# jynik/OOKiedokie

Hardware: NVIDIA B200
Metric: IQ Msamples/s decoded (SC16Q11->OOK msgs) (higher is better)
Workload: dtype f32

## Files before the change

### ookiedokie_b200/csrc/screen_tma.cuh

```cuda
#pragma once

#include <cuda.h>

#include "fir_kernels.cuh"

namespace ookd {

struct ScreenTmaArgs {
    ScreenArgs s;
    i64 row0_sample;
    uint32_t fast_lo, fast_hi;
};

constexpr int STMA_NT = 256, STMA_SPT = 16, STMA_L = STMA_NT * STMA_SPT;
constexpr int STMA_STAGES = 3;
constexpr int STMA_BODY = STMA_L * 4;
constexpr int STMA8_BOX_ROWS = 8;
constexpr int STMA_HT_MAX = 5;
constexpr int STMA_HIST = 384;
constexpr int STMA_XY_ROWS = STMA_NT + STMA_HT_MAX;
constexpr int STMA_SMEM_BYTES = STMA_STAGES * STMA_BODY + STMA_STAGES * STMA_HIST + STMA_STAGES * STMA_XY_ROWS * 8 + 32;
constexpr int STMA_TUNE_BYTES = 528;
static_assert(4 * (STMA_SMEM_BYTES + STMA_TUNE_BYTES + 1024) <= 228 * 1024, "four CTAs per SM");

#ifndef OOKD_STMA_L2_HINT
#define OOKD_STMA_L2_HINT 0x12F0000000000000ull
#endif
#ifndef OOKD_STMA_MINB
#define OOKD_STMA_MINB 4
#endif

__device__ __forceinline__ uint32_t smem_u32(const void *p)
{
    return (uint32_t) __cvta_generic_to_shared(p);
}

__device__ __forceinline__ void mbar_init(uint32_t bar, uint32_t count)
{
    asm volatile("mbarrier.init.shared::cta.b64 [%0], %1;" ::"r"(bar), "r"(count) : "memory");
}

__device__ __forceinline__ void mbar_expect_tx(uint32_t bar, uint32_t bytes)
{
    asm volatile("mbarrier.arrive.expect_tx.shared::cta.b64 _, [%0], %1;" ::"r"(bar), "r"(bytes) : "memory");
}

__device__ __forceinline__ void mbar_wait(uint32_t bar, uint32_t parity)
{
    asm volatile(
        "{\n\t"
        ".reg .pred p;\n\t"
        "WAIT_%=:\n\t"
        "mbarrier.try_wait.parity.shared::cta.b64 p, [%0], %1;\n\t"
        "@p bra DONE_%=;\n\t"
        "bra WAIT_%=;\n\t"
        "DONE_%=:\n\t"
        "}" ::"r"(bar), "r"(parity) : "memory");
}

__device__ __forceinline__ void tma_load_tile(uint32_t dst, const CUtensorMap *map, int32_t row, uint32_t bar)
{
    asm volatile(
        "cp.async.bulk.tensor.2d.shared::cluster.global.mbarrier::complete_tx::bytes.L2::cache_hint"
        " [%0], [%1, {%3, %4}], [%2], %5;" ::"r"(dst), "l"((uint64_t) map), "r"(bar), "r"(0), "r"(row),
        "l"(OOKD_STMA_L2_HINT)
        : "memory");
}

__device__ __forceinline__ uint4 lds128(uint32_t addr)
{
    uint4 v;
    asm volatile("ld.shared.v4.u32 {%0,%1,%2,%3}, [%4];" : "=r"(v.x), "=r"(v.y), "=r"(v.z), "=r"(v.w) : "r"(addr));
    return v;
}

__device__ __forceinline__ void sts128(uint32_t addr, uint32_t a, uint32_t b, uint32_t c, uint32_t d)
{
    asm volatile("st.shared.v4.u32 [%0], {%1,%2,%3,%4};" ::"r"(addr), "r"(a), "r"(b), "r"(c), "r"(d) : "memory");
}

__device__ __forceinline__ int stma_chunk_off(int u, int v)
{
    const int R = u >> 1;
    return R * 128 + (((((u & 1) << 2) | v) ^ (R & 7)) << 4);
}

__device__ __forceinline__ int dp2a_lo_s16_u8(uint32_t a, uint32_t b, int c)
{
    int d;
    asm("dp2a.lo.s32.u32 %0, %1, %2, %3;" : "=r"(d) : "r"(a), "r"(b), "r"(c));
    return d;
}

__device__ __forceinline__ int dp2a_hi_s16_s8(uint32_t a, uint32_t b, int c)
{
    int d;
    asm("dp2a.hi.s32.s32 %0, %1, %2, %3;" : "=r"(d) : "r"(a), "r"(b), "r"(c));
    return d;
}

__device__ __forceinline__ void screen_span_energy(const uint32_t (&w)[16], uint32_t (&pre)[16], uint32_t &hi_total)
{
    int lo = 0, hi = 0;
#pragma unroll
    for (int e = 0; e < 16; e++) {
        const uint32_t b = __byte_perm(w[e], 0u, 0x3120);
        lo = dp2a_lo_s16_u8(w[e], b, lo);
        hi = dp2a_hi_s16_s8(w[e], b, hi);
        pre[e] = (uint32_t) (lo + (hi << 8));
    }
    hi_total = (uint32_t) hi;
}

__device__ __forceinline__ void screen_span_sums(const uint32_t (&w)[16], int &sx, int &sy)
{
    int xs = 0, ys = 0;
#pragma unroll
    for (int e = 0; e < 16; e++) {
        xs += (int) (short) (w[e] & 0xFFFFu);
        ys += ((int) w[e]) >> 16;
    }
    sx = xs;
    sy = ys;
}

#define OOKD_XY_QUIET ((int) 0x80000000)

__device__ __forceinline__ void screen_span_stats_v2(const uint32_t (&w)[16], uint32_t (&pre)[16], int &sx, int &sy, uint32_t &tot,
                                                     uint32_t k0)
{
    uint32_t hi_total;
    screen_span_energy(w, pre, hi_total);
    tot = (hi_total >= (1u << 20)) ? 0xFFFFFFFFu : pre[15];
    if (tot >= k0) {
        screen_span_sums(w, sx, sy);
    } else {
        sx = OOKD_XY_QUIET;
        sy = 0;
    }
}

template <int FMT>
__device__ __forceinline__ void screen_span_stats8(const uint32_t (&x)[8], uint32_t (&pre)[16], int &sx, int &sy,
                                                   uint32_t &tot, uint32_t k0)
{
    uint32_t acc = 0;
#pragma unroll
    for (int j = 0; j < 8; j++) {
#pragma unroll
        for (int h = 0; h < 2; h++) {
            const uint32_t half = h ? 0xFFFF0000u : 0x0000FFFFu;
            const int e = 2 * j + h;
            if constexpr (FMT == FMT_CU8) {
                acc = __dp4a(x[j], ~x[j] & half, acc);
                pre[e] = 8323200u * (uint32_t) (e + 1) - 256u * acc;
            } else {
                acc = (uint32_t) __dp4a((int) x[j], (int) (x[j] & half), (int) acc);
                pre[e] = acc << 8;
            }
        }
    }
    tot = pre[15];
    if (tot >= k0) {
        int xs = 0, ys = 0;
#pragma unroll
        for (int j = 0; j < 8; j++) {
            if constexpr (FMT == FMT_CU8) {
                xs = (int) __dp4a(x[j], 0x00010001u, (uint32_t) xs);
                ys = (int) __dp4a(x[j], 0x01000100u, (uint32_t) ys);
            } else {
                xs = __dp4a((int) x[j], 0x00010001, xs);
                ys = __dp4a((int) x[j], 0x01000100, ys);
            }
        }
        sx = (FMT == FMT_CU8) ? 16 * xs - 16 * 2040 : 16 * xs;
        sy = (FMT == FMT_CU8) ? 16 * ys - 16 * 2040 : 16 * ys;
    } else {
        sx = OOKD_XY_QUIET;
        sy = 0;
    }
}

template <int DEC, bool ADAPT, int FMT>
__global__ void __maxnreg__(64)
fir_screen_tma_kernel(const __grid_constant__ CUtensorMap tmap, const ScreenTmaArgs ta, const ScreenParams sp,
                      const uint32_t tune_step)
{
    static_assert(DEC == 1 || DEC == 4, "shapes with a screening proof");
    constexpr int NT = STMA_NT, SPT = STMA_SPT, L = STMA_L, NS = STMA_STAGES;
    constexpr int HT = (DEC == 1) ? 2 : 5;
    constexpr int LOUT = L / DEC;
    constexpr int LOG_RS = (fmt_raw(FMT) == FMT_SC16Q11) ? 5 : 6;
    extern __shared__ __align__(1024) uint8_t smem_raw[];

    const ScreenArgs &sa = ta.s;
    const TiledArgs &a = sa.t;
    const uint32_t per = (sa.n_tiles + gridDim.x - 1) / gridDim.x;
    const uint32_t t_begin = sa.tile_offset + blockIdx.x * per;
    const uint32_t t_end = min(sa.tile_offset + sa.n_tiles, t_begin + per);
    if (t_begin >= t_end) return;
    if constexpr (ADAPT) {
        if (sa.work_count[OOKD_MODE_SLOT] != OOKD_MODE_ENERGY) return;
    }

    const uint32_t body0 = smem_u32(smem_raw);
    const bool smem_aligned = (body0 & 1023u) == 0;
    const uint32_t hist0 = body0 + NS * STMA_BODY + STMA_HIST;
    const uint32_t xy0 = body0 + NS * STMA_BODY + NS * STMA_HIST;
    const uint32_t bar0 = xy0 + NS * STMA_XY_ROWS * 8;
    const uint32_t tab0 = bar0 + 32;

    const int u = (int) threadIdx.x;
    if (u == 0) {
#pragma unroll
        for (int s = 0; s < NS; s++) mbar_init(bar0 + 8 * s, 1);
        asm volatile("fence.mbarrier_init.release.cluster;" ::: "memory");
    }
    if constexpr (fmt_tuned(FMT)) {
        if (u < 129) asm volatile("st.shared.u32 [%0], %1;" ::"r"(tab0 + 4 * u), "r"(__ldg(tune_pairs + u)) : "memory");
    }
    __syncthreads();

    auto tile_fast = [&](uint32_t tile) -> bool { return smem_aligned && tile >= ta.fast_lo && tile < ta.fast_hi; };
    auto tile_in0 = [&](uint32_t tile) -> i64 { return (a.out_lo + (i64) tile * LOUT) * DEC; };
    auto tile_row = [&](uint32_t tile) -> int32_t { return (int32_t) ((tile_in0(tile) - ta.row0_sample) >> LOG_RS); };
    auto issue = [&](uint32_t tile, int s) {
        const uint32_t bar = bar0 + 8 * s;
        mbar_expect_tx(bar, L * in_bytes<FMT>());
        if constexpr (fmt_raw(FMT) == FMT_SC16Q11) {
            tma_load_tile(body0 + s * STMA_BODY, &tmap, tile_row(tile), bar);
        } else {
#pragma unroll
            for (int w = 0; w < NT / 32; w++) {
                tma_load_tile(body0 + s * STMA_BODY + 2048 * w, &tmap, tile_row(tile) + STMA8_BOX_ROWS * w, bar);
            }
        }
    };
    auto load_span_slow = [&](i64 g, uint32_t (&w)[16]) {
#pragma unroll
        for (int e = 0; e < 16; e++) {
            const i64 ge = g + e;
            w[e] = (ge >= 0 && ge >= a.in_base && ge < a.in_valid_end) ? load_word<FMT>(a.in, ge - a.in_base, ge, tune_step) : 0u;
        }
    };
    auto tune_span = [&](i64 g, uint32_t (&w)[16]) {
        const uint32_t phi0 = (uint32_t) g * tune_step;
#pragma unroll
        for (int e = 0; e < 16; e++) {
            const uint32_t phi = phi0 + (uint32_t) e * tune_step;
            uint32_t pair;
            asm volatile("ld.shared.u32 %0, [%1];" : "=r"(pair) : "r"(tab0 + 4 * tune_row(phi)));
            w[e] = tune_rotate(w[e], phi, pair);
        }
    };
    auto row_base = [&](int s, int uu) -> uint32_t { return (uu >= 0) ? body0 + s * STMA_BODY : hist0 + s * STMA_HIST; };
    auto store_row = [&](int s, int uu, const uint32_t (&p)[16], int xs, int ys) {
        const uint32_t rb = row_base(s, uu);
#pragma unroll
        for (int v = 0; v < 4; v++) {
            sts128(rb + stma_chunk_off(uu, v), p[4 * v], p[4 * v + 1], p[4 * v + 2], p[4 * v + 3]);
        }
        asm volatile("st.shared.v2.u32 [%0], {%1,%2};" ::"r"(xy0 + (s * STMA_XY_ROWS + uu + HT) * 8), "r"(xs), "r"(ys)
                     : "memory");
    };

    if (u == 0) {
        if (tile_fast(t_begin)) issue(t_begin, 0);
        if (t_begin + 1 < t_end && tile_fast(t_begin + 1)) issue(t_begin + 1, 1);
    }
    if (u < HT) {
        uint32_t w[16], p[16];
        int xs, ys;
        load_span_slow(tile_in0(t_begin) - HT * SPT + (i64) u * SPT, w);
        uint32_t tot;
        screen_span_stats_v2(w, p, xs, ys, tot, sp.k0);
        p[15] = tot;
        store_row(0, u - HT, p, xs, ys);
    }

    int off_own[4];
#pragma unroll
    for (int v = 0; v < 4; v++) off_own[v] = stma_chunk_off(u, v);
    auto elem_off = [&](int uu, int e) -> int { return stma_chunk_off(uu, e >> 2) + 4 * (e & 3); };

    int s = 0;
    uint32_t phases = 0;
    for (uint32_t tile = t_begin; tile < t_end; tile++) {
        const uint32_t body = body0 + s * STMA_BODY;
        const uint32_t hist = hist0 + s * STMA_HIST;
        const i64 o0 = a.out_lo + (i64) tile * LOUT;
        uint32_t pre[SPT], tot_own;
        int sx, sy;
        if constexpr (fmt_raw(FMT) == FMT_SC16Q11) {
            uint32_t w[16];
            if (tile_fast(tile)) {
                mbar_wait(bar0 + 8 * s, (phases >> s) & 1u);
                phases ^= 1u << s;
#pragma unroll
                for (int v = 0; v < 4; v++) {
                    const uint4 x = lds128(body + off_own[v]);
                    w[4 * v] = x.x; w[4 * v + 1] = x.y; w[4 * v + 2] = x.z; w[4 * v + 3] = x.w;
                }
                if constexpr (fmt_tuned(FMT)) tune_span(tile_in0(tile) + (i64) u * SPT, w);
            } else {
                load_span_slow(tile_in0(tile) + (i64) u * SPT, w);
            }
            screen_span_stats_v2(w, pre, sx, sy, tot_own, sp.k0);
        } else {
            if (tile_fast(tile)) {
                mbar_wait(bar0 + 8 * s, (phases >> s) & 1u);
                phases ^= 1u << s;
                const int r = (u & 31) >> 2;
                const uint32_t blk = body + 2048 * (u >> 5);
                if constexpr (fmt_tuned(FMT)) {
                    uint32_t w[16];
#pragma unroll
                    for (int v = 0; v < 2; v++) {
                        uint32_t (&w8)[8] = *reinterpret_cast<uint32_t (*)[8]>(w + 8 * v);
                        widen8x8<fmt_raw(FMT)>(lds128(blk + r * 128 + ((((u & 3) << 1 | v) ^ r) << 4)), w8);
                    }
                    tune_span(tile_in0(tile) + (i64) u * SPT, w);
                    screen_span_stats_v2(w, pre, sx, sy, tot_own, sp.k0);
                } else {
                    uint32_t x[8];
#pragma unroll
                    for (int v = 0; v < 2; v++) {
                        const uint4 c = lds128(blk + r * 128 + ((((u & 3) << 1 | v) ^ r) << 4));
                        x[4 * v] = c.x; x[4 * v + 1] = c.y; x[4 * v + 2] = c.z; x[4 * v + 3] = c.w;
                    }
                    screen_span_stats8<FMT>(x, pre, sx, sy, tot_own, sp.k0);
                }
            } else {
                uint32_t w[16];
                load_span_slow(tile_in0(tile) + (i64) u * SPT, w);
                screen_span_stats_v2(w, pre, sx, sy, tot_own, sp.k0);
            }
            __syncwarp();
        }
        {
            uint32_t p[16];
#pragma unroll
            for (int e = 0; e < 15; e++) p[e] = pre[e];
            p[15] = tot_own;
            store_row(s, u, p, sx, sy);
            if (u >= NT - HT) {
                store_row(s == NS - 1 ? 0 : s + 1, u - NT, p, sx, sy);
            }
        }
        asm volatile("fence.proxy.async.shared::cta;" ::: "memory");
        __syncthreads();
        if (u == 0 && tile + 2 < t_end && tile_fast(tile + 2)) {
            issue(tile + 2, s == 0 ? NS - 1 : s - 1);
        }
        auto nb_base = [&](int k) -> uint32_t { return (u < k) ? hist : body; };

        if constexpr (DEC == 1) {
            uint32_t p2[SPT];
#pragma unroll
            for (int v = 0; v < 4; v++) {
                const uint4 x = lds128(nb_base(2) + stma_chunk_off(u - 2, v));
                p2[4 * v] = x.x; p2[4 * v + 1] = x.y; p2[4 * v + 2] = x.z; p2[4 * v + 3] = x.w;
            }
            uint32_t tot1;
            asm volatile("ld.shared.u32 %0, [%1];" : "=r"(tot1) : "r"(nb_base(1) + elem_off(u - 1, 15)));
            const uint32_t tot2 = p2[SPT - 1];
            uint32_t bits16 = 0;
            bool undecided_lo = true, undecided_hi = true;
            const i64 o = o0 + (i64) u * SPT;
            if ((int) (tot_own | tot1 | tot2) >= 0) {
                const uint32_t bsum = tot2 + tot1;
                int dmax_lo = INT_MIN, dmax_hi = INT_MIN;
#pragma unroll
                for (int j = 0; j < SPT; j++) {
                    const int d = (int) (pre[j] - p2[j]);
                    if (j < 8) dmax_lo = max(dmax_lo, d); else dmax_hi = max(dmax_hi, d);
                }
                const bool off_lo = (uint32_t) ((int) bsum + dmax_lo) < sp.k0, off_hi = (uint32_t) ((int) bsum + dmax_hi) < sp.k0;
                bool on = false;
                if (!(off_lo && off_hi)) {
                    int x1, y1, x2, y2;
                    const uint32_t xy = xy0 + (s * STMA_XY_ROWS + u) * 8;
                    asm volatile("ld.shared.v2.u32 {%0,%1}, [%2];" : "=r"(x2), "=r"(y2) : "r"(xy));
                    asm volatile("ld.shared.v2.u32 {%0,%1}, [%2];" : "=r"(x1), "=r"(y1) : "r"(xy + 8));
                    const float X = (float) (sx + x1 + x2), Y = (float) (sy + y1 + y2);
                    const float Q = (float) (bsum + pre[SPT - 1]);
                    const float m2 = fmaf(X, X, Y * Y);
                    const float mu = sqrt_approx(m2) * sp.inv_n;
                    const float V = fmaxf(fmaf(-m2, sp.inv_n, Q), 0.0f) + 1e-5f * Q;
                    const float bc = fmaf(sp.t2, sqrt_approx(V), sp.cg * sqrt_approx(Q));
                    on = fmaf(mu, sp.g_lo, -bc) * 0.99999f > sp.theta_hi;
                    if (sx == OOKD_XY_QUIET || x1 == OOKD_XY_QUIET || x2 == OOKD_XY_QUIET) on = false;
                }
                if (on) {
                    bits16 = 0xFFFFu;
                    undecided_lo = undecided_hi = false;
                } else {
                    undecided_lo = !off_lo;
                    undecided_hi = !off_hi;
                }
            }
            const bool in_lo = o < a.out_hi, in_hi = o + 8 < a.out_hi;
            if (in_lo) {
                const i64 byte = (o - a.bit_base) >> 3;
                if (in_hi) {
                    *(uint16_t *) (a.out_bits + byte) = (uint16_t) bits16;
                } else {
                    a.out_bits[byte] = (uint8_t) bits16;
                }
            }
            const bool push_lo = undecided_lo && in_lo, push_hi = undecided_hi && in_hi;
            const uint32_t m_lo = __ballot_sync(0xFFFFFFFFu, push_lo), m_hi = __ballot_sync(0xFFFFFFFFu, push_hi);
            if (m_lo | m_hi) {
                const uint32_t n_push = __popc(m_lo) + __popc(m_hi);
                const int lane = u & 31;
                uint32_t slot0 = 0;
                if (lane == 0) slot0 = atomicAdd(sa.work_count, n_push);
                slot0 = __shfl_sync(0xFFFFFFFFu, slot0, 0);
                const uint32_t below = (1u << lane) - 1;
                const uint32_t grp0 = (uint32_t) ((o - a.bit_base) >> 3);
                if (push_lo) {
                    const uint32_t sl = slot0 + __popc(m_lo & below);
                    if (sl < sa.work_cap) sa.work_list[sl] = grp0;
                }
                if (push_hi) {
                    const uint32_t sl = slot0 + __popc(m_lo) + __popc(m_hi & below);
                    if (sl < sa.work_cap) sa.work_list[sl] = grp0 + 1;
                }
            }
        } else {
            auto ld = [&](int k, int e) -> uint32_t {
                uint32_t v;
                asm volatile("ld.shared.u32 %0, [%1];" : "=r"(v) : "r"(nb_base(k) + elem_off(u - k, e)));
                return v;
            };
            const uint32_t t1 = ld(1, 15), t2 = ld(2, 15), t3 = ld(3, 15), t4 = ld(4, 15), t5 = ld(5, 15);
            uint32_t bits4 = 0, und = 0xF;
            if ((int) (tot_own | t1 | t2 | t3 | t4 | t5) >= 0) {
                const uint32_t p4_1 = ld(4, 1), p5_5 = ld(5, 5), p5_9 = ld(5, 9), p5_13 = ld(5, 13);
                const uint32_t mid3 = t3 + t2 + t1;
                const uint32_t mid4 = mid3 + t4;
                const uint32_t e0 = (t5 - p5_5) + mid4 + pre[3];
                const uint32_t e1 = (t5 - p5_9) + mid4 + pre[7];
                const uint32_t e2 = (t5 - p5_13) + mid4 + pre[11];
                const uint32_t e3 = (t4 - p4_1) + mid3 + pre[15];
                und = (e0 < sp.k0 ? 0u : 1u) | (e1 < sp.k0 ? 0u : 2u) | (e2 < sp.k0 ? 0u : 4u) | (e3 < sp.k0 ? 0u : 8u);
                if (und) {
                    int X = sx, Y = sy;
                    bool quiet = sx == OOKD_XY_QUIET;
#pragma unroll
                    for (int k = 1; k <= 5; k++) {
                        int xk, yk;
                        asm volatile("ld.shared.v2.u32 {%0,%1}, [%2];" : "=r"(xk), "=r"(yk)
                                     : "r"(xy0 + (s * STMA_XY_ROWS + u - k + HT) * 8));
                        X += xk;
                        Y += yk;
                        quiet = quiet || (xk == OOKD_XY_QUIET);
                    }
                    const float Xf = (float) X, Yf = (float) Y;
                    const float Q = (float) (t5 + mid4 + pre[15]);
                    const float m2 = fmaf(Xf, Xf, Yf * Yf);
                    const float mu = sqrt_approx(m2) * sp.inv_n;
                    const float V = fmaxf(fmaf(-m2, sp.inv_n, Q), 0.0f) + 1e-5f * Q;
                    const float bc = fmaf(sp.t2, sqrt_approx(V), sp.cg * sqrt_approx(Q));
                    if (!quiet && fmaf(mu, sp.g_lo, -bc) * 0.99999f > sp.theta_hi) {
                        bits4 = 0xF;
                        und = 0;
                    }
                }
            }
            const uint32_t other_bits = __shfl_down_sync(0xFFFFFFFFu, bits4, 1);
            const uint32_t other_und = __shfl_down_sync(0xFFFFFFFFu, und, 1);
            const i64 o = o0 + (i64) u * 4;
            const bool in_range = ((u & 1) == 0) && o < a.out_hi;
            const bool push = in_range && ((und | other_und) != 0);
            if (in_range) {
                a.out_bits[(o - a.bit_base) >> 3] = (uint8_t) (bits4 | (other_bits << 4));
            }
            const uint32_t m_push = __ballot_sync(0xFFFFFFFFu, push);
            if (m_push) {
                const int lane = u & 31;
                uint32_t slot0 = 0;
                if (lane == 0) slot0 = atomicAdd(sa.work_count, (uint32_t) __popc(m_push));
                slot0 = __shfl_sync(0xFFFFFFFFu, slot0, 0);
                if (push) {
                    const uint32_t sl = slot0 + __popc(m_push & ((1u << lane) - 1));
                    if (sl < sa.work_cap) sa.work_list[sl] = (uint32_t) ((o - a.bit_base) >> 3);
                }
            }
        }
        s = (s == NS - 1) ? 0 : s + 1;
    }
}

}
```

Measured before the change: 1.002 million.

## Replace per-tile __syncthreads with per-warp mbarrier handoffs and empty/full ring

Drops the block-wide __syncthreads per tile. Each warp now signals its boundary rows through per-warp ready mbarriers, and the next warp (or warp 0 of the next tile) waits only on its predecessor. Slot reuse for TMA loads is governed by empty/full barrier pairs, and the separate history buffer is removed by reading halo rows from the previous stage's slot. Neighbour totals now come through warp shuffles instead of shared loads. This lets warps run ahead of each other, at the cost of more complex barrier and phase bookkeeping and a risk of ordering bugs at stage wraparound.

```diff
diff --git a/ookiedokie_b200/csrc/screen_tma.cuh b/ookiedokie_b200/csrc/screen_tma.cuh
--- a/ookiedokie_b200/csrc/screen_tma.cuh
+++ b/ookiedokie_b200/csrc/screen_tma.cuh
@@ -13,13 +13,13 @@
 };
 
 constexpr int STMA_NT = 256, STMA_SPT = 16, STMA_L = STMA_NT * STMA_SPT;
+constexpr int STMA_WARPS = STMA_NT / 32;
 constexpr int STMA_STAGES = 3;
 constexpr int STMA_BODY = STMA_L * 4;
 constexpr int STMA8_BOX_ROWS = 8;
-constexpr int STMA_HT_MAX = 5;
-constexpr int STMA_HIST = 384;
-constexpr int STMA_XY_ROWS = STMA_NT + STMA_HT_MAX;
-constexpr int STMA_SMEM_BYTES = STMA_STAGES * STMA_BODY + STMA_STAGES * STMA_HIST + STMA_STAGES * STMA_XY_ROWS * 8 + 32;
+constexpr int STMA_XY = STMA_NT * 8;
+constexpr int STMA_BARS = (2 * STMA_STAGES + STMA_STAGES * STMA_WARPS) * 8;
+constexpr int STMA_SMEM_BYTES = STMA_STAGES * (STMA_BODY + STMA_XY) + STMA_BARS;
 constexpr int STMA_TUNE_BYTES = 528;
 static_assert(4 * (STMA_SMEM_BYTES + STMA_TUNE_BYTES + 1024) <= 228 * 1024, "four CTAs per SM");
 
@@ -43,6 +43,11 @@
 __device__ __forceinline__ void mbar_expect_tx(uint32_t bar, uint32_t bytes)
 {
     asm volatile("mbarrier.arrive.expect_tx.shared::cta.b64 _, [%0], %1;" ::"r"(bar), "r"(bytes) : "memory");
+}
+
+__device__ __forceinline__ void mbar_arrive(uint32_t bar)
+{
+    asm volatile("mbarrier.arrive.shared::cta.b64 _, [%0];" ::"r"(bar) : "memory");
 }
 
 __device__ __forceinline__ void mbar_wait(uint32_t bar, uint32_t parity)
@@ -187,10 +192,11 @@
                       const uint32_t tune_step)
 {
     static_assert(DEC == 1 || DEC == 4, "shapes with a screening proof");
-    constexpr int NT = STMA_NT, SPT = STMA_SPT, L = STMA_L, NS = STMA_STAGES;
+    constexpr int NT = STMA_NT, NW = STMA_WARPS, SPT = STMA_SPT, L = STMA_L, NS = STMA_STAGES;
     constexpr int HT = (DEC == 1) ? 2 : 5;
     constexpr int LOUT = L / DEC;
     constexpr int LOG_RS = (fmt_raw(FMT) == FMT_SC16Q11) ? 5 : 6;
+    constexpr uint32_t FULL = 0xFFFFFFFFu;
     extern __shared__ __align__(1024) uint8_t smem_raw[];
 
     const ScreenArgs &sa = ta.s;
@@ -205,15 +211,22 @@
 
     const uint32_t body0 = smem_u32(smem_raw);
     const bool smem_aligned = (body0 & 1023u) == 0;
-    const uint32_t hist0 = body0 + NS * STMA_BODY + STMA_HIST;
-    const uint32_t xy0 = body0 + NS * STMA_BODY + NS * STMA_HIST;
-    const uint32_t bar0 = xy0 + NS * STMA_XY_ROWS * 8;
-    const uint32_t tab0 = bar0 + 32;
-
-    const int u = (int) threadIdx.x;
+    const uint32_t xy0 = body0 + NS * STMA_BODY;
+    const uint32_t bar0 = xy0 + NS * STMA_XY;
+    const uint32_t tab0 = bar0 + STMA_BARS;
+    auto full_bar = [&](int s) -> uint32_t { return bar0 + 8 * s; };
+    auto empty_bar = [&](int s) -> uint32_t { return bar0 + 8 * (NS + s); };
+    auto ready_bar = [&](int s, int w) -> uint32_t { return bar0 + 8 * (2 * NS + NW * s + w); };
+
+    const int u = (int) threadIdx.x, warp = u >> 5, lane = u & 31;
     if (u == 0) {
 #pragma unroll
-        for (int s = 0; s < NS; s++) mbar_init(bar0 + 8 * s, 1);
+        for (int s = 0; s < NS; s++) {
+            mbar_init(full_bar(s), 1);
+            mbar_init(empty_bar(s), NW);
+#pragma unroll
+            for (int w = 0; w < NW; w++) mbar_init(ready_bar(s, w), HT);
+        }
         asm volatile("fence.mbarrier_init.release.cluster;" ::: "memory");
     }
     if constexpr (fmt_tuned(FMT)) {
@@ -225,14 +238,13 @@
     auto tile_in0 = [&](uint32_t tile) -> i64 { return (a.out_lo + (i64) tile * LOUT) * DEC; };
     auto tile_row = [&](uint32_t tile) -> int32_t { return (int32_t) ((tile_in0(tile) - ta.row0_sample) >> LOG_RS); };
     auto issue = [&](uint32_t tile, int s) {
-        const uint32_t bar = bar0 + 8 * s;
-        mbar_expect_tx(bar, L * in_bytes<FMT>());
+        mbar_expect_tx(full_bar(s), L * in_bytes<FMT>());
         if constexpr (fmt_raw(FMT) == FMT_SC16Q11) {
-            tma_load_tile(body0 + s * STMA_BODY, &tmap, tile_row(tile), bar);
+            tma_load_tile(body0 + s * STMA_BODY, &tmap, tile_row(tile), full_bar(s));
         } else {
 #pragma unroll
-            for (int w = 0; w < NT / 32; w++) {
-                tma_load_tile(body0 + s * STMA_BODY + 2048 * w, &tmap, tile_row(tile) + STMA8_BOX_ROWS * w, bar);
+            for (int w = 0; w < NW; w++) {
+                tma_load_tile(body0 + s * STMA_BODY + 2048 * w, &tmap, tile_row(tile) + STMA8_BOX_ROWS * w, full_bar(s));
             }
         }
     };
@@ -253,15 +265,13 @@
             w[e] = tune_rotate(w[e], phi, pair);
         }
     };
-    auto row_base = [&](int s, int uu) -> uint32_t { return (uu >= 0) ? body0 + s * STMA_BODY : hist0 + s * STMA_HIST; };
-    auto store_row = [&](int s, int uu, const uint32_t (&p)[16], int xs, int ys) {
-        const uint32_t rb = row_base(s, uu);
+    auto store_row = [&](int s, int t, const uint32_t (&p)[16], int xs, int ys) {
+        const uint32_t rb = body0 + s * STMA_BODY;
 #pragma unroll
         for (int v = 0; v < 4; v++) {
-            sts128(rb + stma_chunk_off(uu, v), p[4 * v], p[4 * v + 1], p[4 * v + 2], p[4 * v + 3]);
-        }
-        asm volatile("st.shared.v2.u32 [%0], {%1,%2};" ::"r"(xy0 + (s * STMA_XY_ROWS + uu + HT) * 8), "r"(xs), "r"(ys)
-                     : "memory");
+            sts128(rb + stma_chunk_off(t, v), p[4 * v], p[4 * v + 1], p[4 * v + 2], p[4 * v + 3]);
+        }
+        asm volatile("st.shared.v2.u32 [%0], {%1,%2};" ::"r"(xy0 + s * STMA_XY + 8 * t), "r"(xs), "r"(ys) : "memory");
     };
 
     if (u == 0) {
@@ -275,30 +285,36 @@
         uint32_t tot;
         screen_span_stats_v2(w, p, xs, ys, tot, sp.k0);
         p[15] = tot;
-        store_row(0, u - HT, p, xs, ys);
-    }
-
-    int off_own[4];
-#pragma unroll
-    for (int v = 0; v < 4; v++) off_own[v] = stma_chunk_off(u, v);
-    auto elem_off = [&](int uu, int e) -> int { return stma_chunk_off(uu, e >> 2) + 4 * (e & 3); };
+        store_row(NS - 1, NT - HT + u, p, xs, ys);
+    }
+    if (lane >= 32 - HT) mbar_arrive(ready_bar(NS - 1, warp));
+    if (lane == 0 && warp > 0) mbar_arrive(empty_bar(NS - 1));
+
+    const int off_own = stma_chunk_off(u, 0);
+    auto elem_off = [&](int t, int e) -> int { return stma_chunk_off(t, e >> 2) + 4 * (e & 3); };
 
     int s = 0;
+    uint32_t lap = 0;
     uint32_t phases = 0;
     for (uint32_t tile = t_begin; tile < t_end; tile++) {
+        const int s_prev = (s == 0) ? NS - 1 : s - 1;
+        const uint32_t lap_prev = (s == NS - 1) ? lap ^ 1u : lap;
         const uint32_t body = body0 + s * STMA_BODY;
-        const uint32_t hist = hist0 + s * STMA_HIST;
         const i64 o0 = a.out_lo + (i64) tile * LOUT;
         uint32_t pre[SPT], tot_own;
         int sx, sy;
+        if (tile_fast(tile)) {
+            mbar_wait(full_bar(s), (phases >> s) & 1u);
+            phases ^= 1u << s;
+        } else if (tile >= t_begin + NS - 1) {
+            mbar_wait(empty_bar(s), lap ^ 1u);
+        }
         if constexpr (fmt_raw(FMT) == FMT_SC16Q11) {
             uint32_t w[16];
             if (tile_fast(tile)) {
-                mbar_wait(bar0 + 8 * s, (phases >> s) & 1u);
-                phases ^= 1u << s;
 #pragma unroll
                 for (int v = 0; v < 4; v++) {
-                    const uint4 x = lds128(body + off_own[v]);
+                    const uint4 x = lds128(body + (off_own ^ (v << 4)));
                     w[4 * v] = x.x; w[4 * v + 1] = x.y; w[4 * v + 2] = x.z; w[4 * v + 3] = x.w;
                 }
                 if constexpr (fmt_tuned(FMT)) tune_span(tile_in0(tile) + (i64) u * SPT, w);
@@ -308,16 +324,14 @@
             screen_span_stats_v2(w, pre, sx, sy, tot_own, sp.k0);
         } else {
             if (tile_fast(tile)) {
-                mbar_wait(bar0 + 8 * s, (phases >> s) & 1u);
-                phases ^= 1u << s;
-                const int r = (u & 31) >> 2;
-                const uint32_t blk = body + 2048 * (u >> 5);
+                const int r = lane >> 2;
+                const uint32_t blk = body + 2048 * warp;
                 if constexpr (fmt_tuned(FMT)) {
                     uint32_t w[16];
 #pragma unroll
                     for (int v = 0; v < 2; v++) {
                         uint32_t (&w8)[8] = *reinterpret_cast<uint32_t (*)[8]>(w + 8 * v);
-                        widen8x8<fmt_raw(FMT)>(lds128(blk + r * 128 + ((((u & 3) << 1 | v) ^ r) << 4)), w8);
+                        widen8x8<fmt_raw(FMT)>(lds128(blk + r * 128 + ((((lane & 3) << 1 | v) ^ r) << 4)), w8);
                     }
                     tune_span(tile_in0(tile) + (i64) u * SPT, w);
                     screen_span_stats_v2(w, pre, sx, sy, tot_own, sp.k0);
@@ -325,7 +339,7 @@
                     uint32_t x[8];
 #pragma unroll
                     for (int v = 0; v < 2; v++) {
-                        const uint4 c = lds128(blk + r * 128 + ((((u & 3) << 1 | v) ^ r) << 4));
+                        const uint4 c = lds128(blk + r * 128 + ((((lane & 3) << 1 | v) ^ r) << 4));
                         x[4 * v] = c.x; x[4 * v + 1] = c.y; x[4 * v + 2] = c.z; x[4 * v + 3] = c.w;
                     }
                     screen_span_stats8<FMT>(x, pre, sx, sy, tot_own, sp.k0);
@@ -343,26 +357,36 @@
             for (int e = 0; e < 15; e++) p[e] = pre[e];
             p[15] = tot_own;
             store_row(s, u, p, sx, sy);
-            if (u >= NT - HT) {
-                store_row(s == NS - 1 ? 0 : s + 1, u - NT, p, sx, sy);
-            }
-        }
-        asm volatile("fence.proxy.async.shared::cta;" ::: "memory");
-        __syncthreads();
-        if (u == 0 && tile + 2 < t_end && tile_fast(tile + 2)) {
-            issue(tile + 2, s == 0 ? NS - 1 : s - 1);
-        }
-        auto nb_base = [&](int k) -> uint32_t { return (u < k) ? hist : body; };
+        }
+        if (lane >= 32 - HT) mbar_arrive(ready_bar(s, warp));
+        __syncwarp();
+        if (lane < HT) {
+            if (warp > 0) {
+                mbar_wait(ready_bar(s, warp - 1), lap);
+            } else {
+                mbar_wait(ready_bar(s_prev, NW - 1), lap_prev);
+            }
+        }
+        auto nb = [&](int k) -> uint32_t { return (u < k) ? body0 + s_prev * STMA_BODY : body; };
+        auto nb_xy = [&](int k) -> uint32_t { return xy0 + (u < k ? s_prev : s) * STMA_XY + 8 * ((u - k) & (NT - 1)); };
+        int u_t = u;
+        if constexpr (DEC == 4) asm volatile("" : "+r"(u_t));
+        auto tot_back = [&](int k) -> uint32_t {
+            uint32_t t = __shfl_sync(FULL, tot_own, (lane - k) & 31);
+            if (lane < k) {
+                asm volatile("ld.shared.u32 %0, [%1];" : "=r"(t) : "r"(nb(k) + elem_off((u_t - k) & (NT - 1), 15)));
+            }
+            return t;
+        };
 
         if constexpr (DEC == 1) {
             uint32_t p2[SPT];
 #pragma unroll
             for (int v = 0; v < 4; v++) {
-                const uint4 x = lds128(nb_base(2) + stma_chunk_off(u - 2, v));
+                const uint4 x = lds128(nb(2) + stma_chunk_off((u - 2) & (NT - 1), v));
                 p2[4 * v] = x.x; p2[4 * v + 1] = x.y; p2[4 * v + 2] = x.z; p2[4 * v + 3] = x.w;
             }
-            uint32_t tot1;
-            asm volatile("ld.shared.u32 %0, [%1];" : "=r"(tot1) : "r"(nb_base(1) + elem_off(u - 1, 15)));
+            const uint32_t tot1 = tot_back(1);
             const uint32_t tot2 = p2[SPT - 1];
             uint32_t bits16 = 0;
             bool undecided_lo = true, undecided_hi = true;
@@ -379,9 +403,8 @@
                 bool on = false;
                 if (!(off_lo && off_hi)) {
                     int x1, y1, x2, y2;
-                    const uint32_t xy = xy0 + (s * STMA_XY_ROWS + u) * 8;
-                    asm volatile("ld.shared.v2.u32 {%0,%1}, [%2];" : "=r"(x2), "=r"(y2) : "r"(xy));
-                    asm volatile("ld.shared.v2.u32 {%0,%1}, [%2];" : "=r"(x1), "=r"(y1) : "r"(xy + 8));
+                    asm volatile("ld.shared.v2.u32 {%0,%1}, [%2];" : "=r"(x2), "=r"(y2) : "r"(nb_xy(2)));
+                    asm volatile("ld.shared.v2.u32 {%0,%1}, [%2];" : "=r"(x1), "=r"(y1) : "r"(nb_xy(1)));
                     const float X = (float) (sx + x1 + x2), Y = (float) (sy + y1 + y2);
                     const float Q = (float) (bsum + pre[SPT - 1]);
                     const float m2 = fmaf(X, X, Y * Y);
@@ -409,13 +432,12 @@
                 }
             }
             const bool push_lo = undecided_lo && in_lo, push_hi = undecided_hi && in_hi;
-            const uint32_t m_lo = __ballot_sync(0xFFFFFFFFu, push_lo), m_hi = __ballot_sync(0xFFFFFFFFu, push_hi);
+            const uint32_t m_lo = __ballot_sync(FULL, push_lo), m_hi = __ballot_sync(FULL, push_hi);
             if (m_lo | m_hi) {
                 const uint32_t n_push = __popc(m_lo) + __popc(m_hi);
-                const int lane = u & 31;
                 uint32_t slot0 = 0;
                 if (lane == 0) slot0 = atomicAdd(sa.work_count, n_push);
-                slot0 = __shfl_sync(0xFFFFFFFFu, slot0, 0);
+                slot0 = __shfl_sync(FULL, slot0, 0);
                 const uint32_t below = (1u << lane) - 1;
                 const uint32_t grp0 = (uint32_t) ((o - a.bit_base) >> 3);
                 if (push_lo) {
@@ -430,10 +452,10 @@
         } else {
             auto ld = [&](int k, int e) -> uint32_t {
                 uint32_t v;
-                asm volatile("ld.shared.u32 %0, [%1];" : "=r"(v) : "r"(nb_base(k) + elem_off(u - k, e)));
+                asm volatile("ld.shared.u32 %0, [%1];" : "=r"(v) : "r"(nb(k) + elem_off((u - k) & (NT - 1), e)));
                 return v;
             };
-            const uint32_t t1 = ld(1, 15), t2 = ld(2, 15), t3 = ld(3, 15), t4 = ld(4, 15), t5 = ld(5, 15);
+            const uint32_t t1 = tot_back(1), t2 = tot_back(2), t3 = tot_back(3), t4 = tot_back(4), t5 = tot_back(5);
             uint32_t bits4 = 0, und = 0xF;
             if ((int) (tot_own | t1 | t2 | t3 | t4 | t5) >= 0) {
                 const uint32_t p4_1 = ld(4, 1), p5_5 = ld(5, 5), p5_9 = ld(5, 9), p5_13 = ld(5, 13);
@@ -450,8 +472,7 @@
 #pragma unroll
                     for (int k = 1; k <= 5; k++) {
                         int xk, yk;
-                        asm volatile("ld.shared.v2.u32 {%0,%1}, [%2];" : "=r"(xk), "=r"(yk)
-                                     : "r"(xy0 + (s * STMA_XY_ROWS + u - k + HT) * 8));
+                        asm volatile("ld.shared.v2.u32 {%0,%1}, [%2];" : "=r"(xk), "=r"(yk) : "r"(nb_xy(k)));
                         X += xk;
                         Y += yk;
                         quiet = quiet || (xk == OOKD_XY_QUIET);
@@ -468,28 +489,37 @@
                     }
                 }
             }
-            const uint32_t other_bits = __shfl_down_sync(0xFFFFFFFFu, bits4, 1);
-            const uint32_t other_und = __shfl_down_sync(0xFFFFFFFFu, und, 1);
+            const uint32_t other_bits = __shfl_down_sync(FULL, bits4, 1);
+            const uint32_t other_und = __shfl_down_sync(FULL, und, 1);
             const i64 o = o0 + (i64) u * 4;
             const bool in_range = ((u & 1) == 0) && o < a.out_hi;
             const bool push = in_range && ((und | other_und) != 0);
             if (in_range) {
                 a.out_bits[(o - a.bit_base) >> 3] = (uint8_t) (bits4 | (other_bits << 4));
             }
-            const uint32_t m_push = __ballot_sync(0xFFFFFFFFu, push);
+            const uint32_t m_push = __ballot_sync(FULL, push);
             if (m_push) {
-                const int lane = u & 31;
                 uint32_t slot0 = 0;
                 if (lane == 0) slot0 = atomicAdd(sa.work_count, (uint32_t) __popc(m_push));
-                slot0 = __shfl_sync(0xFFFFFFFFu, slot0, 0);
+                slot0 = __shfl_sync(FULL, slot0, 0);
                 if (push) {
                     const uint32_t sl = slot0 + __popc(m_push & ((1u << lane) - 1));
                     if (sl < sa.work_cap) sa.work_list[sl] = (uint32_t) ((o - a.bit_base) >> 3);
                 }
             }
         }
+        asm volatile("fence.proxy.async.shared::cta;" ::: "memory");
+        __syncwarp();
+        if (lane == 0) {
+            mbar_arrive(warp > 0 ? empty_bar(s) : empty_bar(s_prev));
+        }
+        if (u == 0 && tile + 2 < t_end && tile_fast(tile + 2)) {
+            mbar_wait(empty_bar(s_prev), lap_prev);
+            issue(tile + 2, s_prev);
+        }
         s = (s == NS - 1) ? 0 : s + 1;
-    }
-}
-
-}
+        if (s == NS - 1) lap ^= 1u;
+    }
+}
+
+}
```

Result: slower. 566,300, median of 6 (-43.5%).
